# msracver/Relation-Networks-for-Object-Detection

Hardware: AMD Instinct MI355X
Metric: images/sec (1000x600, 300 ROIs) (higher is better)
Workload: dtype bf16; 1 GPU; BASELINE configs[1]: ResNet-101 Faster-RCNN + 2 relation modules (N=300, 16 heads, d=1024) + soft-NMS(0.6) + top-100, 600x1000 images, 300 proposals, random-init weights; launch=hipGraph replay, batches_in_flight=1, parallelism=replicas x1 (no data-path collective), ranks_seen_by_rccl=1

## Files before the change

include/relnet_hip.h:

```cpp
#ifndef RELNET_HIP_H
#define RELNET_HIP_H

#ifdef __cplusplus
extern "C" {
#endif

enum { RELNET_F32 = 0, RELNET_BF16 = 1 };

int relnet_version(void);
const char* relnet_last_error(void);
unsigned long long relnet_stream_capture_id(void* stream);

void _nms(int* keep_out, int* num_out, const float* boxes_host, int boxes_num, int boxes_dim,
          float nms_overlap_thresh, int device_id);

int relnet_proposal_decode(const float* cls_prob, const long* cls_strides4, const float* deltas,
                           const long* delta_strides4, const float* im_info, const double* base_anchors,
                           float* boxes , float* scores , int B, int A, int h, int w,
                           int feat_stride, int min_size, int softmax_pairs, void* stream);
int relnet_topk_sort(const float* scores, const float* boxes, float* out_boxes5, int* out_index,
                     int* out_count, int B, int n, int K, void* stream);
int relnet_nms_mask(const float* boxes5, const int* counts , unsigned long long* mask,
                    int B, int n, int n_stride, float thresh, void* stream);
int relnet_nms_scan(const unsigned long long* mask, const float* boxes5, const int* counts, float* rois,
// ... 73 lines not shown

int relnet_geometry_bias(const float* boxes, int box_stride, int box_off, const float* wp_t, const float* bp,
                         const float* divisors8, void* bias, int bias_half , float* pos_mat,
                         float* pos_emb, int B, int N, int M, int Mpad, int fc_dim, int nmod, void* stream);

int relnet_relation_attention(const void* q, long q_ld, long q_bs, const void* k, long k_ld, long k_bs,
                              const void* vwt, long vwt_ld, long vwt_bs, const void* bias, int bias_half,
                              long bias_bs, const float* bout, const void* resid, long resid_ld, long resid_bs, void* out,
                              long out_ld, long out_bs, void* out_act, long act_ld, long act_bs, float* logits,
                              int B, int H, int N, int M, int Mpad, float scale, int in_dtype, int out_dtype,
                              void* stream);

int relnet_relation_attention_kc(const void* q, long q_ld, long q_bs, const void* k, long k_ld, long k_bs,
                                 const void* vwt, long vwt_ld, long vwt_bs, const void* bias, int bias_half,
                                 long bias_bs, const float* bout, const void* resid, long resid_ld, long resid_bs, void* out,
                                 long out_ld, long out_bs, void* out_act, long act_ld, long act_bs, float* logits,
                                 int B, int H, int N, int M, int Mpad, float scale, int in_dtype, int out_dtype,
                                 const int* key_count, void* stream);
void relnet_relation_attention_debug_lds_f32(int on);

int relnet_relation_attention_fused(const void* q, long q_ld, long q_bs, const void* k, long k_ld, long k_bs,
                                    const void* vwt, long vwt_ld, long vwt_bs, const float* boxes, int box_stride,
                                    int box_off, const float* wp, const float* bp, const float* divisors8,
                                    const float* bout, const void* resid, long resid_ld, long resid_bs, void* out,
                                    long out_ld, long out_bs, void* out_act, long act_ld, long act_bs, int B, int H,
                                    int N, int M, int Mpad, float scale, void* stream);

int relnet_bottleneck_chain(const void* mid2, const void* x, const void* w3f, const void* w1f, const float* b3,
                            const float* b1, void* x_next, void* mid1_next, long P, int mid, void* stream);
int relnet_bottleneck_chain_proj(const void* mid2, const void* x_in, const void* w3f, const void* wpf, const void* w1f,
                                 const float* b3p, const float* b1, void* x_next, void* mid1_next, long P, int mid, void* stream);
int relnet_bottleneck_chain_s2(const void* mid2, const void* x, const void* w3f, const float* b3, void* x_next, int B, int H,
                               int W, int mid, void* stream);

int relnet_conv3x3_c64(const void* in, const void* w_frag, const float* bias, int relu, void* out, int B, int H, int W,
                       void* stream);
int relnet_conv3x3_c64_s2(const void* in, const void* w_frag, const float* bias, int relu, void* out, int B, int H, int W,
                          void* stream);


int relnet_pack_w_frag(const void* w, long ldw, void* out, int N, int K, void* stream);
int relnet_conv2d_nhwc_wf(const void* in, long in_pix, long in_img, const void* w, const void* w_frag, const float* bias,
                          const void* resid, int relu, void* out, long ldc, int B, int H, int W, int Cin, int Cout, int R,
                          int S, int stride, int dil, int pad, int out_dtype, void* stream);

int relnet_detect_head(const float* cls_score, long cs_ld, const float* bbox_pred, long bp_ld, const float* rois,
                       const float* im_info, float* cls_prob, double* boxes, int R, int C, int rois_per_image,
                       int delta_off, void* stream);
int relnet_detect_head_ex(const float* cls_score, long cs_ld, const float* bbox_pred, long bp_ld, const float* rois,
                          const float* im_info, float* cls_prob, double* boxes, int R, int C, int rois_per_image,
                          int delta_off, const int* n_valid, void* stream);
int relnet_class_nms(const float* cls_prob, const double* boxes, double* dets, int* counts, int B, int N, int C,
                     float score_thresh, double nms_param, int soft, int max_picks, void* stream);
int relnet_class_nms_ex(const float* cls_prob, const double* scores64, const double* boxes, double* dets, int* counts,
                        int* pick_index, int B, int N, int C, float score_thresh, double nms_param, int soft,
                        int max_picks, void* stream);
int relnet_class_nms_hist_bins(void);
int relnet_class_nms_topk(const float* cls_prob, const double* boxes, double* dets, int* counts, void* hist, int B, int N, int C,
                          float score_thresh, double nms_param, int soft, int max_picks, int top_k, void* stream);
int relnet_image_topk(const double* dets, const int* counts, double* thresh, int* total, float* out,
                      int* out_count, int B, int NC, int N, int max_per_image, int max_out, void* stream);

int relnet_lnms_prepare(const float* cls_score, long cs_ld, const float* bbox_pred, long bp_ld, const float* rois,
                        const float* im_info, float* prob , float* boxes , int B, int N,
                        int C, int delta_off, const float* means4, const float* stds4, void* stream);
int relnet_lnms_prepare_ex(const float* cls_score, long cs_ld, const float* bbox_pred, long bp_ld, const float* rois,
// ... 214 lines not shown
```

relation-networks-for-object-detection_amd/backbone.py:

```python
import math
import os

import torch
import torch.nn.functional as F

from . import ops

UNITS = (3, 4, 23, 3)
FILTERS = (256, 512, 1024, 2048)
EPS = 1e-5
PIXEL_MEANS = (103.06, 115.90, 123.15)


def unit_names(fpn=False):
    out = []
    in_ch = 64
    for si, (n, oc) in enumerate(zip(UNITS, FILTERS)):
        stage = si + 2
        for u in range(n):
            if n <= 3 or stage == 2 or stage == 5:
                name = 'abc'[u]
            else:
                name = 'a' if u == 0 else 'b%d' % u
            stride = 2 if (u == 0 and (stage in (3, 4) or (fpn and stage == 5))) else 1
# ... 51 lines not shown
        p['res5%s_branch2b_offset_weight' % u] = nrm(dcn_offset_std, 72, 512, 3, 3)
        p['res5%s_branch2b_offset_bias' % u] = torch.zeros(72)
    p['offset_weight'] = nrm(dcn_offset_std, 98, 256 * 49); p['offset_bias'] = torch.zeros(98)
    if fpn:
        for lvl, cin in ((32, 2048), (16, 1024), (8, 512), (4, 256)):
            p['fpn_ft%d_1x1_weight' % lvl] = nrm(0.01, 256, cin, 1, 1); p['fpn_ft%d_1x1_bias' % lvl] = torch.zeros(256)
            p['fpn_ft%d_3x3_weight' % lvl] = nrm(0.01, 256, 256, 3, 3); p['fpn_ft%d_3x3_bias' % lvl] = torch.zeros(256)
        p['fpn_ft64_3x3_weight'] = nrm(0.01, 256, 256, 3, 3); p['fpn_ft64_3x3_bias'] = torch.zeros(256)
        p['roi_pool_fc1_weight'] = nrm(0.01, 1024, 256 * 49); p['roi_pool_fc1_bias'] = torch.zeros(1024)
        p['roi_pool_fc2_weight'] = nrm(0.01, 1024, 1024); p['roi_pool_fc2_bias'] = torch.zeros(1024)
    return p


def fold_bn(w, gamma, beta, mean, var, eps=EPS):
    s = gamma.double() / torch.sqrt(var.double() + eps)
    return (w.double() * s.view(-1, 1, 1, 1)).float(), (beta.double() - mean.double() * s).float()


class Backbone(object):

    def __init__(self, params, dtype=torch.bfloat16, device='cuda', channels_last=True, impl=None, stem='hip', dcn=False,
                 fpn=False, chain=True, frozen_only=False, pixel_means=PIXEL_MEANS):
        self.dtype, self.device, self.dcn, self.fpn = dtype, device, dcn, fpn
        self.frozen_only = frozen_only
        self.pixel_means = tuple(float(v) for v in pixel_means)
        self.use_chain = chain
        env = os.environ.get('RELNET_STAGE_SPLIT')
        if env not in (None, '', '0'):
            self.stage_split = {int(a): int(b) for a, b in (kv.split(':') for kv in env.split(','))}
        if os.environ.get('RELNET_INPLACE_EXPAND') is not None:
            self.inplace_expand = os.environ['RELNET_INPLACE_EXPAND'] not in ('', '0')
        if os.environ.get('RELNET_QUARTER_UNITS') is not None:
            self.quarter_units = os.environ['RELNET_QUARTER_UNITS'] not in ('', '0')
        self.impl = impl or ('hip' if dtype == torch.bfloat16 else ('hip32' if dtype == torch.float32 and torch.device(device).type == 'cuda' else 'miopen'))
        if self.impl == 'hip' and torch.device(device).type == 'cuda':
            ops.asm_selfcheck()
        self.stem = stem
        assert self.impl in ('hip', 'hip32', 'miopen') and (self.impl != 'hip' or dtype == torch.bfloat16) and (self.impl != 'hip32' or dtype == torch.float32)
        self.mf = torch.channels_last if channels_last else torch.contiguous_format
        self.w = {}
        self.wp = {}
        self.wf = {}
        self.b32 = {}
        self.wp32 = {}
        for conv, bn, oc, ic, k in conv_bn_names():
            if frozen_only and not conv.startswith(('conv1', 'res2')):
                continue
            w, b = fold_bn(params[conv + '_weight'], params[bn + '_gamma'], params[bn + '_beta'],
                           params[bn + '_moving_mean'], params[bn + '_moving_var'])
            self._put(conv, w, b)
        if frozen_only:
            pass
        elif fpn:
            for lvl in (32, 16, 8, 4):
                for k in ('1x1', '3x3'):
                    name = 'fpn_ft%d_%s' % (lvl, k)
                    self._put(name, params[name + '_weight'], params[name + '_bias'])
        else:
            for name in ('rpn_conv_3x3', 'rpn_cls_score', 'rpn_bbox_pred', 'conv_new_1'):
                self._put(name, params[name + '_weight'], params[name + '_bias'])
            self._put('rpn_out', torch.cat([params['rpn_cls_score_weight'], params['rpn_bbox_pred_weight']], 0),
                      torch.cat([params['rpn_cls_score_bias'], params['rpn_bbox_pred_bias']], 0))
        self.units = [u for u in unit_names(fpn) if not frozen_only or u[0] == 2]
        self.wp_dcn = {}
        if dcn and not frozen_only:
            for u in 'abc':
# ... 54 lines not shown
    def _float_image(self, data, im_info, dtype):
        if data.dtype != torch.uint8:
            return data
        return ops.image_transform_u8(data, self.pixel_means, im_info, dtype=dtype)

    def forward_res2(self, data, im_info=None):
        if self.impl == 'hip32':
            assert self.frozen_only
            return self._forward_hip32(self._float_image(data, im_info, torch.float32))
        x = ops.stem_fused(data, self.w_stem, self.b32['conv1'], im_info, self.pixel_means)
        y_next = None
        self.last_chain_units = []
        for unit in self.units:
            if unit[0] != 2:
                break
            x, y_next = self._unit_hip(x, unit, y_next)
        return x

    def _forward_hip(self, data, rpn_hook=None, im_info=None):
        if self.stem == 'hip':
            x = ops.stem_fused(data, self.w_stem, self.b32['conv1'], im_info, self.pixel_means)
        elif self.stem == 'hip3':
            x = ops.stem_conv7(self._float_image(data, im_info, torch.float32), self.w_stem, self.b32['conv1'], relu=True)
            x = ops.stem_bias_relu_pool(x, self.zero_bias64)
        else:
            x = self._float_image(data, im_info, torch.float32).to(self.dtype).contiguous(memory_format=self.mf)
            x = F.conv2d(x, self.w['conv1'][0], None, stride=2, padding=3)
            x = ops.stem_bias_relu_pool(x.permute(0, 2, 3, 1), self.b32['conv1'])
        conv4 = None
        ends = {}
        y_next = None
        side, hooked = None, None
        self.last_chain_units, self.last_side_stream, self.last_stage_split = [], False, {}
        self.last_quarter_units = []
        compact = False
        ui = 0
        while ui < len(self.units):
            unit = self.units[ui]
            stage, proj = unit[0], unit[7]
            if stage == 5 and conv4 is None:
                conv4 = x
                if rpn_hook is not None and not self.fpn:
                    main = torch.cuda.current_stream()
                    side = self._side_stream()
                    self.last_side_stream = True
                    side.wait_stream(main)
                    with torch.cuda.stream(side):
                        hooked = self._rpn_head(conv4)
                        hooked = hooked + (rpn_hook(hooked[0], hooked[1]),)
            if proj and stage > 2:
                ends[stage - 1] = x
            nsplit = self._stage_split(stage, x, unit) if proj else 1
            if nsplit > 1:
                stage_units = [u for u in self.units if u[0] == stage]
                x = self._run_stage_split(x, stage_units, nsplit)
                ui += len(stage_units)
                continue
            quarter = self._quarter_ok(x, unit, self.units[ui + 1] if ui + 1 < len(self.units) else None)
            x, y_next = self._unit_hip(x, unit, y_next, inplace=self.inplace_expand, quarter=quarter, subsampled=compact)
            compact = quarter
            ui += 1
        conv5 = x
        nchw = lambda t: t.permute(0, 3, 1, 2)
        if self.fpn:
            tops = {32: self._hconv(conv5, 'fpn_ft32_1x1')}
            for lvl, src in ((16, ends[4]), (8, ends[3]), (4, ends[2])):
                tops[lvl] = ops.upsample2x_add_(self._hconv(src, 'fpn_ft%d_1x1' % lvl), tops[lvl * 2])
            out = {'fpn_ft%d' % lvl: nchw(self._hconv(tops[lvl], 'fpn_ft%d_3x3' % lvl, pad=1)) for lvl in (4, 8, 16, 32)}
            out.update(conv4=nchw(conv4), conv5=nchw(conv5))
            return out
        feat = self._hconv(conv5, 'conv_new_1', relu=True)
        out = dict(conv4=nchw(conv4), conv5=nchw(conv5), conv_new_1_relu=nchw(feat))
        if hooked is not None:
            torch.cuda.current_stream().wait_stream(side)
            out.update(rpn_cls_score=hooked[0], rpn_bbox_pred=hooked[1], rpn_hook=hooked[2])
        else:
            out['rpn_cls_score'], out['rpn_bbox_pred'] = self._rpn_head(conv4)
        return out

    stage_split = None
    inplace_expand = True

    quarter_units = True

    def _quarter_ok(self, x, unit, nxt):
        stage, nm, ic, mc, oc, stride, dil, proj = unit
        if not self.quarter_units or self.fpn or nxt is None or nxt[0] != stage + 1 or nxt[5] != 2 or not nxt[7]:
            return False
        ch = self.chain.get(nm)
        if ch is None or ch[1] is not None or mc not in ops.CHAIN_S2_MIDS or proj or dil != 1 or (self.dcn and stage == 5):
            return False
        if mc in ops.HALO3_CHANNELS and ('res%s_branch2b' % nm) not in self.halo3:
            return False
        if self.stage_split and (self._stage_split(stage, x, unit) > 1 or self._stage_split(nxt[0], x, nxt) > 1):
            return False
        B, H, W, C = x.shape
        return C == oc and x.numel() * 2 < (1 << 32) and ops.chain_worthwhile(B * ((H - 1) // 2 + 1) * ((W - 1) // 2 + 1), mc)

    def _stage_split(self, stage, x, unit):
        return int(self.stage_split.get(stage, 1)) if self.stage_split else 1

    def _run_stage_split(self, x, stage_units, nsplit):
        B = x.shape[0]
        stage = stage_units[0][0]
        st, nm, ic, mc, oc, stride, dil, proj = stage_units[0]
        Ho, Wo = (x.shape[1] - 1) // stride + 1, (x.shape[2] - 1) // stride + 1
        out = torch.empty((B, Ho, Wo, oc), device=x.device, dtype=x.dtype)
        bounds = [(B * i) // nsplit for i in range(nsplit + 1)]
        self.last_stage_split[stage] = [hi - lo for lo, hi in zip(bounds, bounds[1:])]
        for lo, hi in zip(bounds, bounds[1:]):
            xs, ys = x[lo:hi], None
            for unit in stage_units:
                xs, ys = self._unit_hip(xs, unit, ys, sc_out=out[lo:hi] if unit[7] else None, inplace=self.inplace_expand, force_chain=True)
            if xs.data_ptr() != out[lo:hi].data_ptr():
                out[lo:hi].copy_(xs)
        return out

    def _unit_hip(self, x, unit, y_pre=None, sc_out=None, inplace=False, force_chain=False, quarter=False, subsampled=False):
        stage, nm, ic, mc, oc, stride, dil, proj = unit
        if subsampled:
            assert stride == 2 and proj
            stride = 1
        if quarter:
            y = y_pre if y_pre is not None else self._hconv(x, 'res%s_branch2a' % nm, relu=True)
            if ('res%s_branch2b' % nm) in self.halo3:
                y = ops.conv3x3_halo_s2(y.contiguous(), *self.halo3['res%s_branch2b' % nm], relu=True)
            else:
                y = self._hconv(y, 'res%s_branch2b' % nm, stride=2, pad=1, relu=True)
            w3f, _, b3, _ = self.chain[nm]
            if nm not in self.last_chain_units:
                self.last_chain_units.append(nm)
            self.last_quarter_units.append(nm)
            return ops.bottleneck_chain_s2(y, x.contiguous(), w3f, b3), None
        fuse_proj = (nm in self.chain_proj and sc_out is None and x.is_contiguous()
                     and (force_chain or ops.chain_worthwhile(x.numel() // x.shape[-1], mc)))
        if fuse_proj:
            sc = None
        elif proj:
            w, b, k = self.wp['res%s_branch1' % nm]
            sc = ops.conv2d_nhwc(x, w, b, ksize=k, stride=stride, out=sc_out)
        else:
            sc = x
        y = y_pre if y_pre is not None else self._hconv(x, 'res%s_branch2a' % nm, stride=stride, relu=True)
        if self.dcn and stage == 5:
            y = self._deform_2b(y.permute(0, 3, 1, 2), 'res%s_branch2b' % nm,
                                self._hconv(y, 'res%s_branch2b_offset' % nm, pad=2, dil=2, out_dtype=torch.float32).permute(0, 3, 1, 2))
            y = y.permute(0, 2, 3, 1)
        elif ('res%s_branch2b' % nm) in self.halo3:
            y = ops.conv3x3_halo(y.contiguous(), *self.halo3['res%s_branch2b' % nm], relu=True)
        else:
            y = self._hconv(y, 'res%s_branch2b' % nm, pad=dil, dil=dil, relu=True)
        if fuse_proj:
            if nm not in self.last_chain_units:
                self.last_chain_units.append(nm)
            return ops.bottleneck_chain_proj(y, x, *self.chain_proj[nm])
        ch = self.chain.get(nm)
        if ch is not None and not force_chain and not ops.chain_worthwhile(y.numel() // y.shape[-1], y.shape[-1]):
            ch = None
        if ch is not None:
            if nm not in self.last_chain_units:
                self.last_chain_units.append(nm)
            return ops.bottleneck_chain(y, sc.contiguous(), *ch, inplace=inplace and sc.is_contiguous())
        return self._hconv(y, 'res%s_branch2c' % nm, relu=True, resid=sc), None

    def _rpn_head(self, conv4):
        r = self._hconv(conv4, 'rpn_conv_3x3', pad=1, relu=True)
        rpn = self._hconv(r, 'rpn_out', out_dtype=torch.float32)
        na2 = self.w['rpn_cls_score'][0].shape[0]
        return rpn[..., :na2].permute(0, 3, 1, 2), rpn[..., na2:].permute(0, 3, 1, 2)

    def _side_stream(self):
        if getattr(self, '_side', None) is None:
            self._side = torch.cuda.Stream(device=self.device)
        return self._side

    def _deform_2b(self, y, name, offset):
        w, b = self.wp_dcn[name]
        return ops.deformable_conv(y, offset, w, b, 3, 1, 2, 2, 4, relu=True)

    def _conv(self, x, name, stride=1, pad=0, dil=1, relu=False):
        w, b = self.w[name]
        y = F.conv2d(x, w, b, stride=stride, padding=pad, dilation=dil)
        return F.relu_(y) if relu else y

    def _c32(self, x, name, stride=1, pad=0, dil=1, relu=False, resid=None):
        w, b, k = self.wp32[name]
        return ops.conv2d_nhwc_f32(x, w, b, ksize=k, stride=stride, pad=pad, dil=dil, relu=relu, resid=resid)

    def _forward_hip32(self, data):
        B, Cin, H, W = data.shape
        x = torch.zeros((B, H, W, 16), device=data.device, dtype=torch.float32)
        x[..., :Cin] = data.permute(0, 2, 3, 1)
        x = self._c32(x, 'conv1', stride=2, pad=3, relu=True)
        x = ops.maxpool_nhwc_f32(x, 3, 2)
        conv4, ends = None, {}
# ... 70 lines not shown
```

relation-networks-for-object-detection_amd/csrc/bottleneck.hip:

```cpp
#include "common.h"

namespace relnet {

typedef const __attribute__((address_space(1))) void* gas_ptr;
typedef __attribute__((address_space(3))) void* las_ptr;

__device__ __forceinline__ void chain_glds16(const void* src, unsigned lds_byte_addr) {
  asm volatile("s_mov_b32 m0, %1\n\ts_nop 0\n\tglobal_load_lds_dwordx4 %0, off" ::"v"(src), "s"(lds_byte_addr) : "memory", "m0");
}

struct ChainArgs {
  const unsigned short* m2;
  const unsigned short* x;
  const uint4* w3f;
  const uint4* w1f;
  const float* b3;
  const float* b1;
  const unsigned short* xin;
  const uint4* wpf;
  unsigned short* xn;
  unsigned short* m1;
  int P;
  int H, W, Ho, Wo;
  int dbg;
};

template <int MID, bool STREAM, bool REDUCE = true, int KSPLIT = 1, bool PROJ = false, bool GATHER = false>
__global__ __launch_bounds__(512) void bottleneck_chain_kernel(ChainArgs a) {
  static_assert(!PROJ || (!STREAM && KSPLIT == 1), "the projection form exists for the resident-weight kernel");
  static_assert(!GATHER || (!REDUCE && !PROJ && KSPLIT == 1), "the stride-2 gather exists for the plain expand-only forms");
  static_assert(KSPLIT == 1 || (STREAM && !REDUCE), "k-split passes exist for the streamed expand-only form");
  constexpr int COUT = 4 * MID, KS = MID / 16, KSS = KS / KSPLIT, RT = MID / 32, NP = COUT / 64;
  static_assert(!REDUCE || MID <= 128, "MID = 256 with the second product is chain256_roles_kernel");
  constexpr int W3P = 2 * KSS * 1024, W1P = REDUCE ? 4 * RT * 1024 : 0;
  constexpr int WPP = PROJ ? W3P : 0;
  constexpr int PASSB = W3P + WPP + W1P;
  constexpr int STG = PROJ ? 4096 : 8192;
  constexpr int WBYTES = STREAM ? 2 * PASSB : NP * PASSB;
  extern __shared__ __attribute__((aligned(16))) unsigned char smem[];
  const int tid = threadIdx.x, lane = tid & 63;
  const int wave = __builtin_amdgcn_readfirstlane(tid >> 6);
  const int half = lane >> 5, l31 = lane & 31;
  unsigned char* stage = smem + WBYTES + wave * STG;
  float* sB3 = (float*)(smem + WBYTES + 8 * STG);
  float* sB1 = sB3 + COUT;
  for (int i = tid; i < COUT; i += 512) sB3[i] = a.b3[i];
  if constexpr (REDUCE) for (int i = tid; i < MID; i += 512) sB1[i] = a.b1[i];
  if constexpr (!STREAM) {
    for (int i = tid; i < NP * PASSB / 16; i += 512) {
      const int p = i / (PASSB / 16), r = i % (PASSB / 16);
      uint4 v;
      if (r < W3P / 16) v = a.w3f[(long)p * (W3P / 16) + r];
      else if (r < (W3P + WPP) / 16) v = a.wpf[(long)p * (W3P / 16) + (r - W3P / 16)];
      else { const int q = (r - (W3P + WPP) / 16) >> 6, rt = q >> 2, kk = q & 3; v = a.w1f[((long)rt * (COUT / 16) + p * 4 + kk) * 64 + (r & 63)]; }
      ((uint4*)smem)[i] = v;
    }
  }
  __syncthreads();
  const int ntile = (a.P + 31) / 32;
  const int drow = lane >> 3, dslot = lane & 7;
  unsigned xrow[GATHER ? 4 : 1];
  auto gather_rows = [&](int p0) {
    if constexpr (GATHER) {
      const unsigned hw = (unsigned)(a.Ho * a.Wo);
#pragma unroll
      for (int i = 0; i < 4; ++i) {
        const unsigned q = (unsigned)min(p0 + 8 * i + drow, a.P - 1);
        const unsigned b = q / hw, r = q - b * hw, yo = r / (unsigned)a.Wo, xo = r - yo * (unsigned)a.Wo;
        xrow[i] = ((b * (unsigned)a.H + 2u * yo) * (unsigned)a.W + 2u * xo) * (COUT * 2u);
      }
    }
  };
  auto issue_x = [&](int p0, int p) {
    if constexpr (PROJ) return;
    unsigned char* sb = stage + (p & 1) * 4096;
#pragma unroll
    for (int i = 0; i < 4; ++i) {
      const int row = 8 * i + drow;
      const unsigned off = GATHER ? xrow[i] + (p * 64 + ((dslot ^ ((row >> 1) & 7)) << 3)) * 2u
                                  : ((unsigned)min(p0 + row, a.P - 1) * COUT + p * 64 + ((dslot ^ ((row >> 1) & 7)) << 3)) * 2u;
      __builtin_amdgcn_global_load_lds((gas_ptr)((const unsigned char*)a.x + off), (las_ptr)(sb + i * 1024), 16, 0, 0);
    }
  };
  auto issue_w = [&](int st) {
    if constexpr (STREAM) {
      const int p = st / KSPLIT, kh = st % KSPLIT;
      unsigned char* wb = smem + (st & 1) * PASSB;
#pragma unroll
      for (int i = 0; i < (2 * KSS + (REDUCE ? 4 * RT : 0)) / 8; ++i) {
        const int q = wave + 8 * i;
        if (q < 2 * KSS) {
          const int ct = q / KSS, ks = q % KSS;
          __builtin_amdgcn_global_load_lds((gas_ptr)(a.w3f + ((long)((p * 2 + ct) * KS + kh * KSS + ks) * 64 + lane)), (las_ptr)(wb + q * 1024), 16, 0, 0);
        } else {
          const int q1 = q - 2 * KSS, rt = q1 >> 2, kk = q1 & 3;
          __builtin_amdgcn_global_load_lds((gas_ptr)(a.w1f + ((long)(rt * (COUT / 16) + p * 4 + kk) * 64 + lane)), (las_ptr)(wb + W3P + q1 * 1024), 16, 0, 0);
        }
      }
    }
  };
  auto flush = [&](int p0, int p) {
    const unsigned char* sb = stage + (PROJ ? 0 : (p & 1) * 4096) + lane * 16;
    const uint4 v0 = *(const uint4*)sb, v1 = *(const uint4*)(sb + 1024), v2 = *(const uint4*)(sb + 2048), v3 = *(const uint4*)(sb + 3072);
    asm volatile("s_waitcnt lgkmcnt(0)" ::: "memory");
    auto put = [&](int i, const uint4& v) {
      const int row = 8 * i + drow;
      if (p0 + row < a.P) *(uint4*)((unsigned char*)a.xn + ((unsigned)(p0 + row) * COUT + p * 64 + ((dslot ^ ((row >> 1) & 7)) << 3)) * 2u) = v;
    };
    put(0, v0); put(1, v1); put(2, v2); put(3, v3);
  };

  const int t_first = blockIdx.x * 8 + wave;
  const int t_step = gridDim.x * 8;
  const int n_iter = STREAM ? ((ntile + 7) / 8 - (int)blockIdx.x + (int)gridDim.x - 1) / (int)gridDim.x
                            : (ntile - t_first + t_step - 1) / t_step;
  if (n_iter <= 0) return;
  gather_rows(t_first * 32);
  issue_x(t_first * 32, 0);
  issue_w(0);
  for (int it = 0; it < n_iter; ++it) {
    const int p0 = (t_first + it * t_step) * 32;
    const int px = min(p0 + l31, a.P - 1);
    bf16x8 m2f[KS];
#pragma unroll
    for (int ks = 0; ks < KS; ++ks) m2f[ks] = *(const bf16x8*)(a.m2 + (long)px * MID + 16 * ks + 8 * half);
    bf16x8 xf[PROJ ? KS : 1];
    if constexpr (PROJ) {
#pragma unroll
      for (int ks = 0; ks < KS; ++ks) xf[ks] = *(const bf16x8*)(a.xin + (long)px * MID + 16 * ks + 8 * half);
    }
    f32x16 m1acc[RT];
#pragma unroll
    for (int rt = 0; rt < RT; ++rt)
#pragma unroll
      for (int r = 0; r < 16; ++r) m1acc[rt][r] = 0.f;
#pragma unroll 1
    for (int p = 0; p < NP; ++p) {
      f32x16 acc[2];
#pragma unroll
      for (int kh = 0; kh < KSPLIT; ++kh) {
        const int st = p * KSPLIT + kh;
        if constexpr (STREAM) asm volatile("s_waitcnt vmcnt(0)\n\ts_barrier" ::: "memory");
        else if constexpr (!PROJ) asm volatile("s_waitcnt vmcnt(0)" ::: "memory");
        if (kh == 0) {
          if (!PROJ && p > 0) flush(p0, p - 1);
          if (p + 1 < NP) issue_x(p0, p + 1);
          else if (it + 1 < n_iter) { gather_rows(p0 + t_step * 32); issue_x(p0 + t_step * 32, 0); }
        }
        if (st + 1 < NP * KSPLIT) issue_w(st + 1);
        else if (it + 1 < n_iter) issue_w(0);
        const uint4* w3 = (const uint4*)(smem + (STREAM ? (st & 1) : st) * PASSB);
#pragma unroll
        for (int ct = 0; ct < 2; ++ct) {
          if (kh == 0)
#pragma unroll
// ... 305 lines not shown
    else if (mid == 128) bottleneck_chain_kernel<128, true, false><<<grid, 512, lds, (hipStream_t)stream>>>(a);
    else if (mid == 256) bottleneck_chain_kernel<256, true, false><<<grid, 512, lds, (hipStream_t)stream>>>(a);
    else bottleneck_chain_kernel<512, true, false, 2><<<grid, 512, lds, (hipStream_t)stream>>>(a);
  }
  return check_launch("relnet_bottleneck_chain");
}

extern "C" int relnet_bottleneck_chain_s2(const void* mid2, const void* x, const void* w3f, const float* b3, void* x_next, int B,
                                          int H, int W, int mid, void* stream) {
  RELNET_REQUIRE(mid2 && x && w3f && b3 && x_next && x_next != x, "relnet_bottleneck_chain_s2: null operand (or x_next == x: this form is never in place)");
  RELNET_REQUIRE(mid == 64 || mid == 128, "relnet_bottleneck_chain_s2: mid = %d unsupported (64, 128)", mid);
  RELNET_REQUIRE(B > 0 && H > 0 && W > 0 && (long)B * H * W * 8 * mid < (1L << 32),
                 "relnet_bottleneck_chain_s2: bad geometry B=%d H=%d W=%d (the full 4 mid-channel map must stay below 4 GiB)", B, H, W);
  ChainArgs a;
  a.m2 = (const unsigned short*)mid2; a.x = (const unsigned short*)x; a.w3f = (const uint4*)w3f; a.w1f = nullptr;
  a.b3 = b3; a.b1 = nullptr; a.xn = (unsigned short*)x_next; a.m1 = nullptr;
  a.xin = nullptr; a.wpf = nullptr; a.dbg = 0;
  a.H = H; a.W = W; a.Ho = (H - 1) / 2 + 1; a.Wo = (W - 1) / 2 + 1;
  const long P = (long)B * a.Ho * a.Wo;
  a.P = (int)P;
  static relnet::PerDeviceOnce attr_once;
  if (attr_once.first()) {
    hipFuncSetAttribute((const void*)bottleneck_chain_kernel<64, false, false, 1, false, true>, hipFuncAttributeMaxDynamicSharedMemorySize, 160 * 1024);
    hipFuncSetAttribute((const void*)bottleneck_chain_kernel<128, true, false, 1, false, true>, hipFuncAttributeMaxDynamicSharedMemorySize, 160 * 1024);
  }
  const long ntile = (P + 31) / 32;
  const unsigned grid = (unsigned)(ntile < 8 * 256 ? (ntile + 7) / 8 : 256);
  const size_t lds = 65536 + 65536 + (size_t)5 * mid * 4;
  if (mid == 64) bottleneck_chain_kernel<64, false, false, 1, false, true><<<grid, 512, lds, (hipStream_t)stream>>>(a);
  else bottleneck_chain_kernel<128, true, false, 1, false, true><<<grid, 512, lds, (hipStream_t)stream>>>(a);
  return check_launch("relnet_bottleneck_chain_s2");
}

extern "C" int relnet_bottleneck_chain_proj(const void* mid2, const void* x_in, const void* w3f, const void* wpf, const void* w1f,
                                            const float* b3p, const float* b1, void* x_next, void* mid1_next, long P, int mid,
                                            void* stream) {
  RELNET_REQUIRE(mid2 && x_in && w3f && wpf && b3p && x_next, "relnet_bottleneck_chain_proj: null operand");
  RELNET_REQUIRE((w1f && b1 && mid1_next) || (!w1f && !b1 && !mid1_next), "relnet_bottleneck_chain_proj: w1f, b1 and mid1_next are given together (or all NULL)");
  RELNET_REQUIRE(mid == 64, "relnet_bottleneck_chain_proj: mid = %d unsupported (64)", mid);
  RELNET_REQUIRE(P > 0 && P * 8 * mid < (1L << 32), "relnet_bottleneck_chain_proj: bad pixel count %ld (x_next is addressed with 32-bit byte offsets: the 4 mid-channel map must stay below 4 GiB)", P);
  ChainArgs a;
  a.m2 = (const unsigned short*)mid2; a.x = nullptr; a.w3f = (const uint4*)w3f; a.w1f = (const uint4*)w1f;
  a.b3 = b3p; a.b1 = b1; a.xn = (unsigned short*)x_next; a.m1 = (unsigned short*)mid1_next; a.P = (int)P;
  a.xin = (const unsigned short*)x_in; a.wpf = (const uint4*)wpf; a.dbg = 0;
  a.H = a.W = a.Ho = a.Wo = 0;
  static relnet::PerDeviceOnce attr_once;
  if (attr_once.first()) {
    hipFuncSetAttribute((const void*)bottleneck_chain_kernel<64, false, true, 1, true>, hipFuncAttributeMaxDynamicSharedMemorySize, 160 * 1024);
    hipFuncSetAttribute((const void*)bottleneck_chain_kernel<64, false, false, 1, true>, hipFuncAttributeMaxDynamicSharedMemorySize, 160 * 1024);
  }
  const long ntile = (P + 31) / 32;
  const unsigned grid = (unsigned)(ntile < 8 * 256 ? (ntile + 7) / 8 : 256);
  const size_t lds = (size_t)4 * (8192 + 8192 + (mid1_next ? 8192 : 0)) + 8 * 4096 + (size_t)5 * mid * 4;
  if (mid1_next) bottleneck_chain_kernel<64, false, true, 1, true><<<grid, 512, lds, (hipStream_t)stream>>>(a);
  else bottleneck_chain_kernel<64, false, false, 1, true><<<grid, 512, lds, (hipStream_t)stream>>>(a);
  return check_launch("relnet_bottleneck_chain_proj");
}

namespace relnet {

__device__ __attribute__((aligned(16))) const unsigned int g_zero_chunk[4] = {0u, 0u, 0u, 0u};

struct Halo3Args {
  const unsigned short* in;
  const uint4* wf;
  const float* bias;
// ... 178 lines not shown
```

relation-networks-for-object-detection_amd/lib.py:

```python
import ctypes as C
import os
import sys

HERE = os.path.dirname(os.path.abspath(__file__))
LIB_PATH = os.environ.get('RELNET_LIB') or os.path.join(HERE, 'librelnet_hip.so')

F32, BF16 = 0, 1


class RelnetError(RuntimeError):
    pass


_lib = None

_vp, _i, _l, _f, _d = C.c_void_p, C.c_int, C.c_long, C.c_float, C.c_double

_SIGNATURES = {
    'relnet_version': (C.c_int, []),
    'relnet_last_error': (C.c_char_p, []),
    'relnet_gemm_nt': (C.c_int, [_vp, _l, _l, _vp, _l, _l, _vp, _l, _l, _vp, _i, _vp, _i,
                                 _i, _i, _i, _i, _i, _i, _vp]),
    'relnet_geometry_bias': (C.c_int, [_vp, _i, _i, _vp, _vp, _vp, _vp, _i, _vp, _vp, _i, _i, _i, _i,
                                       _i, _i, _vp]),
    'relnet_relation_attention': (C.c_int, [_vp, _l, _l, _vp, _l, _l, _vp, _l, _l, _vp, _i, _l, _vp,
                                            _vp, _l, _l, _vp, _l, _l, _vp, _l, _l, _vp,
                                            _i, _i, _i, _i, _i, _f, _i, _i, _vp]),
    'relnet_relation_attention_kc': (C.c_int, [_vp, _l, _l, _vp, _l, _l, _vp, _l, _l, _vp, _i, _l, _vp,
                                               _vp, _l, _l, _vp, _l, _l, _vp, _l, _l, _vp,
                                               _i, _i, _i, _i, _i, _f, _i, _i, _vp, _vp]),
    'relnet_relation_attention_fused': (C.c_int, [_vp, _l, _l, _vp, _l, _l, _vp, _l, _l, _vp, _i, _i, _vp, _vp, _vp,
                                                  _vp, _vp, _l, _l, _vp, _l, _l, _vp, _l, _l,
                                                  _i, _i, _i, _i, _i, _f, _vp]),
    'relnet_bottleneck_chain': (C.c_int, [_vp, _vp, _vp, _vp, _vp, _vp, _vp, _vp, _l, _i, _vp]),
    'relnet_bottleneck_chain_proj': (C.c_int, [_vp, _vp, _vp, _vp, _vp, _vp, _vp, _vp, _vp, _l, _i, _vp]),
    'relnet_conv3x3_c64': (C.c_int, [_vp, _vp, _vp, _i, _vp, _i, _i, _i, _vp]),
    'relnet_conv3x3_c64_s2': (C.c_int, [_vp, _vp, _vp, _i, _vp, _i, _i, _i, _vp]),
    'relnet_bottleneck_chain_s2': (C.c_int, [_vp, _vp, _vp, _vp, _vp, _i, _i, _i, _i, _vp]),
    'relnet_proposal_decode': (C.c_int, [_vp, _vp, _vp, _vp, _vp, _vp, _vp, _vp, _i, _i, _i, _i, _i, _i, _i, _vp]),
    'relnet_topk_sort': (C.c_int, [_vp, _vp, _vp, _vp, _vp, _i, _i, _i, _vp]),
    'relnet_nms_mask': (C.c_int, [_vp, _vp, _vp, _i, _i, _i, _f, _vp]),
    'relnet_nms_scan': (C.c_int, [_vp, _vp, _vp, _vp, _vp, _vp, _vp, _i, _i, _i, _i, _i, _i, _vp]),
    '_nms': (None, [_vp, _vp, _vp, _i, _i, _f, _i]),
    'relnet_roi_pool_fwd': (C.c_int, [_vp, _vp, _vp, _vp, _vp, _vp, _i, _i, _i, _i, _i, _i, _f, _i, _i, _vp]),
    'relnet_roi_align_fwd': (C.c_int, [_vp, _vp, _vp, _vp, _vp, _i, _i, _i, _i, _i, _i, _f, _i, _i, _i, _i, _vp]),
    'relnet_roi_align_bwd': (C.c_int, [_vp, _vp, _vp, _vp, _vp, _i, _i, _i, _i, _i, _i, _f, _i, _i, _i, _i, _vp]),
    'relnet_roi_align_levels_fwd': (C.c_int, [_vp, _vp, _vp, _vp, _vp, _i, _vp, _vp, _vp, _vp] + [_i] * 9 + [_vp]),
    'relnet_roi_align_levels_bwd': (C.c_int, [_vp, _vp, _vp, _vp, _vp, _vp, _vp, _vp, _vp] + [_i] * 10 + [_vp]),
    'relnet_roi_pool_bwd': (C.c_int, [_vp, _vp, _vp, _vp, _vp, _l, _l, _i, _i, _i, _i, _i, _i, _i, _vp]),
    'relnet_roi_pool_bwd_ex': (C.c_int, [_vp, _vp, _vp, _vp, _vp, _l, _l, _l, _i, _i, _i, _i, _i, _i, _i, _vp]),
    'relnet_roi_pool_fpn_bwd_ex': (C.c_int, [_vp, _vp, _vp, _vp, _vp, _vp, _vp, _vp, _vp, _i, _i, _i, _i, _i, _i, _i, _vp]),
    'relnet_detect_head': (C.c_int, [_vp, _l, _vp, _l, _vp, _vp, _vp, _vp, _i, _i, _i, _i, _vp]),
    'relnet_detect_head_ex': (C.c_int, [_vp, _l, _vp, _l, _vp, _vp, _vp, _vp, _i, _i, _i, _i, _vp, _vp]),
    'relnet_class_nms': (C.c_int, [_vp, _vp, _vp, _vp, _i, _i, _i, _f, C.c_double, _i, _i, _vp]),
    'relnet_class_nms_ex': (C.c_int, [_vp, _vp, _vp, _vp, _vp, _vp, _i, _i, _i, _f, C.c_double, _i, _i, _vp]),
    'relnet_class_nms_topk': (C.c_int, [_vp, _vp, _vp, _vp, _vp, _i, _i, _i, _f, C.c_double, _i, _i, _i, _vp]),
    'relnet_class_nms_hist_bins': (C.c_int, []),
    'relnet_bbox_overlaps': (C.c_int, [_vp, _vp, _vp, _i, _i, _vp]),
    'relnet_image_topk': (C.c_int, [_vp, _vp, _vp, _vp, _vp, _vp, _i, _i, _i, _i, _i, _vp]),
    'relnet_conv2d_nhwc': (C.c_int, [_vp, _l, _l, _vp, _vp, _vp, _i, _vp, _l, _i, _i, _i, _i, _i, _i, _i, _i, _i, _i, _i, _vp]),
    'relnet_conv2d_nhwc_f32': (C.c_int, [_vp, _l, _l, _vp, _vp, _vp, _i, _vp, _l, _i, _i, _i, _i, _i, _i, _i, _i, _i, _i, _vp]),
    'relnet_maxpool_nhwc_f32': (C.c_int, [_vp, _vp, _i, _i, _i, _i, _i, _i, _vp]),
    'relnet_pack_w_frag': (C.c_int, [_vp, _l, _vp, _i, _i, _vp]),
    'relnet_conv2d_nhwc_wf': (C.c_int, [_vp, _l, _l, _vp, _vp, _vp, _vp, _i, _vp, _l, _i, _i, _i, _i, _i, _i, _i, _i, _i, _i, _i, _vp]),
    'relnet_deformable_im2col': (C.c_int, [_vp, _vp, _vp, _vp, _vp, _l] + [_i] * 15 + [_vp]),
    'relnet_deformable_psroi_pool_fwd': (C.c_int, [_vp, _vp, _vp, _vp, _vp, _vp, _vp] + [_i] * 9 + [_f, _f, _i, _i, _i, _vp]),
    'relnet_roi_pool_fpn_fwd': (C.c_int, [_vp, _vp, _vp, _vp, _vp, _i, _vp, _vp, _vp, _vp, _vp, _i, _i, _i, _i, _i, _i, _vp]),
    'relnet_fpn_roi_dispatch': (C.c_int, [_vp, _i, _i, _vp, _vp, _vp, _vp, _i, _i, _i, _vp]),
    'relnet_fpn_roi_dispatch_ex': (C.c_int, [_vp, _i, _i, _vp, _vp, _vp, _vp, _i, _i, _i, _vp, _i, _i, _vp, _vp]),
    'relnet_upsample2x_add': (C.c_int, [_vp, _vp, _i, _i, _i, _i, _i, _vp]),
    'relnet_softmax_output': (C.c_int, [_vp, _vp, _vp, _vp, _vp, _l, _i, _l, _i, _f, _f, _vp]),
# ... 149 lines not shown
```

relation-networks-for-object-detection_amd/ops.py:

```python
import math
import os

import torch

from . import lib as _lib

F32, BF16 = _lib.F32, _lib.BF16


def _dt(t):
    if t.dtype == torch.float32:
        return F32
    if t.dtype == torch.bfloat16:
        return BF16
    raise TypeError("unsupported dtype %s (float32 or bfloat16)" % t.dtype)


def _chk(*ts):
    for t in ts:
        if t is not None:
            if not t.is_cuda:
                raise _lib.RelnetError("relnet ops need GPU tensors (HIP kernels only; no CPU fallback)")


# ... 565 lines not shown
    row = rt * 32 + (lane & 31)
    col = ks * 16 + 8 * (t >> 2) + 4 * (lane >> 5) + (t & 3)
    return w_packed[row, col].contiguous()


def bottleneck_chain(mid2, x, w3_frag, w1_frag, b3, b1, inplace=False):
    _chk(mid2, x, w3_frag, w1_frag, b3, b1)
    mid = mid2.shape[-1]
    assert mid2.is_contiguous() and x.is_contiguous() and x.shape[-1] == 4 * mid and x.shape[:-1] == mid2.shape[:-1]
    assert mid2.dtype == torch.bfloat16 and x.dtype == torch.bfloat16 and b3.dtype == torch.float32
    assert (w1_frag is None) == (b1 is None) and (b1 is None or b1.dtype == torch.float32)
    assert mid in (CHAIN_MIDS if w1_frag is not None else CHAIN_EXPAND_MIDS)
    xn = x if inplace else torch.empty_like(x)
    m1 = torch.empty_like(mid2) if w1_frag is not None else None
    _lib.call('relnet_bottleneck_chain', mid2.data_ptr(), x.data_ptr(), w3_frag.data_ptr(), _ptr(w1_frag), b3.data_ptr(),
              _ptr(b1), xn.data_ptr(), _ptr(m1), mid2.numel() // mid, mid, _stream())
    return xn, m1


CHAIN_S2_MIDS = (64, 128)


def bottleneck_chain_s2(mid2, x, w3_frag, b3):
    _chk(mid2, x, w3_frag, b3)
    mid = mid2.shape[-1]
    B, H, W, C = x.shape
    assert mid in CHAIN_S2_MIDS and C == 4 * mid and mid2.shape == (B, (H - 1) // 2 + 1, (W - 1) // 2 + 1, mid)
    assert mid2.is_contiguous() and x.is_contiguous() and x.numel() * 2 < (1 << 32)
    assert mid2.dtype == torch.bfloat16 and x.dtype == torch.bfloat16 and b3.dtype == torch.float32
    xn = torch.empty(mid2.shape[:-1] + (C,), device=x.device, dtype=x.dtype)
    _lib.call('relnet_bottleneck_chain_s2', mid2.data_ptr(), x.data_ptr(), w3_frag.data_ptr(), b3.data_ptr(), xn.data_ptr(), B, H, W, mid,
              _stream())
    return xn


def bottleneck_chain_proj(mid2, x_in, w3_frag, wp_frag, w1_frag, b3p, b1):
    _chk(mid2, x_in, w3_frag, wp_frag, w1_frag, b3p, b1)
    mid = mid2.shape[-1]
    assert mid == 64 and x_in.shape == mid2.shape and mid2.is_contiguous() and x_in.is_contiguous()
    assert mid2.dtype == torch.bfloat16 and x_in.dtype == torch.bfloat16 and b3p.dtype == torch.float32
    assert (w1_frag is None) == (b1 is None)
    xn = torch.empty(mid2.shape[:-1] + (4 * mid,), device=mid2.device, dtype=torch.bfloat16)
    m1 = torch.empty_like(mid2) if w1_frag is not None else None
    _lib.call('relnet_bottleneck_chain_proj', mid2.data_ptr(), x_in.data_ptr(), w3_frag.data_ptr(), wp_frag.data_ptr(), _ptr(w1_frag),
              b3p.data_ptr(), _ptr(b1), xn.data_ptr(), _ptr(m1), mid2.numel() // mid, mid, _stream())
    return xn, m1


def conv2d_nhwc(x, w_packed, bias, ksize=1, stride=1, pad=0, dil=1, relu=False, resid=None, out=None,
                out_dtype=None, w_frag=None):
    _chk(x, w_packed, bias, resid, out)
    if x.dtype == torch.float32:
        return conv2d_nhwc_f32(x, w_packed, bias, ksize, stride, pad, dil, relu, resid, out)
    assert x.dtype == torch.bfloat16 and w_packed.dtype == torch.bfloat16 and x.stride(3) == 1
    B, H, W, Cin = x.shape
    assert x.stride(1) == W * x.stride(2), "rows of an image must be dense in W"
    Cout = w_packed.shape[0]
    assert w_packed.shape[1] == ksize * ksize * Cin and w_packed.is_contiguous()
    Hout = (H + 2 * pad - dil * (ksize - 1) - 1) // stride + 1
    Wout = (W + 2 * pad - dil * (ksize - 1) - 1) // stride + 1
    odt = out_dtype or (out.dtype if out is not None else x.dtype)
    if out is None:
        out = torch.empty((B, Hout, Wout, Cout), device=x.device, dtype=odt)
    assert out.shape == (B, Hout, Wout, Cout) and out.stride(3) == 1
    assert out.stride(1) == Wout * out.stride(2) and out.stride(0) == Hout * out.stride(1)
    if resid is not None:
# ... 745 lines not shown
```

Before: 2983 images/s.

## Store only even-pixel outputs from the chain kernel preceding a stride-2 quarter unit

Adds an EVEN variant of the fused bottleneck chain kernel. When the following unit is a stride-2 quarter unit, it writes the expanded output x_next only at even (y,x) pixels into a compact subsampled map, while still producing the full mid1 map for the next unit. The next quarter unit then reads this compact map as its shortcut through the plain chain kernel instead of gathering it with stride 2. The intent is to cut three quarters of the full-resolution write of the 4*mid-channel activation and the strided gather that followed it. In exchange the kernel does extra per-row index arithmetic, and the Python scheduling becomes more coupled because each unit now depends on the two units after it.

```diff
diff --git a/include/relnet_hip.h b/include/relnet_hip.h
--- a/include/relnet_hip.h
+++ b/include/relnet_hip.h
@@ -129,6 +129,8 @@
                                  const float* b3p, const float* b1, void* x_next, void* mid1_next, long P, int mid, void* stream);
 int relnet_bottleneck_chain_s2(const void* mid2, const void* x, const void* w3f, const float* b3, void* x_next, int B, int H,
                                int W, int mid, void* stream);
+int relnet_bottleneck_chain_even(const void* mid2, const void* x, const void* w3f, const void* w1f, const float* b3, const float* b1,
+                                 void* x_next_even, void* mid1_next, int B, int H, int W, int mid, void* stream);
 
 int relnet_conv3x3_c64(const void* in, const void* w_frag, const float* bias, int relu, void* out, int B, int H, int W,
                        void* stream);
diff --git a/relation-networks-for-object-detection_amd/backbone.py b/relation-networks-for-object-detection_amd/backbone.py
--- a/relation-networks-for-object-detection_amd/backbone.py
+++ b/relation-networks-for-object-detection_amd/backbone.py
@@ -107,6 +107,8 @@
             self.inplace_expand = os.environ['RELNET_INPLACE_EXPAND'] not in ('', '0')
         if os.environ.get('RELNET_QUARTER_UNITS') is not None:
             self.quarter_units = os.environ['RELNET_QUARTER_UNITS'] not in ('', '0')
+        if os.environ.get('RELNET_EVEN_STORE') is not None:
+            self.even_store = os.environ['RELNET_EVEN_STORE'] not in ('', '0')
         self.impl = impl or ('hip' if dtype == torch.bfloat16 else ('hip32' if dtype == torch.float32 and torch.device(device).type == 'cuda' else 'miopen'))
         if self.impl == 'hip' and torch.device(device).type == 'cuda':
             ops.asm_selfcheck()
@@ -227,8 +229,9 @@
         y_next = None
         side, hooked = None, None
         self.last_chain_units, self.last_side_stream, self.last_stage_split = [], False, {}
-        self.last_quarter_units = []
+        self.last_quarter_units, self.last_even_store_units = [], []
         compact = False
+        even_prev = False
         ui = 0
         while ui < len(self.units):
             unit = self.units[ui]
@@ -251,9 +254,12 @@
                 x = self._run_stage_split(x, stage_units, nsplit)
                 ui += len(stage_units)
                 continue
-            quarter = self._quarter_ok(x, unit, self.units[ui + 1] if ui + 1 < len(self.units) else None)
-            x, y_next = self._unit_hip(x, unit, y_next, inplace=self.inplace_expand, quarter=quarter, subsampled=compact)
-            compact = quarter
+            after = lambda k: self.units[ui + k] if ui + k < len(self.units) else None
+            quarter = even_prev or self._quarter_ok(x, unit, after(1))
+            even = not quarter and self._even_store_ok(x, unit, after(1), after(2))
+            x, y_next = self._unit_hip(x, unit, y_next, inplace=self.inplace_expand, quarter=quarter, subsampled=compact,
+                                       even_store=even, compact_shortcut=even_prev)
+            compact, even_prev = quarter, even
             ui += 1
         conv5 = x
         nchw = lambda t: t.permute(0, 3, 1, 2)
@@ -292,6 +298,17 @@
         B, H, W, C = x.shape
         return C == oc and x.numel() * 2 < (1 << 32) and ops.chain_worthwhile(B * ((H - 1) // 2 + 1) * ((W - 1) // 2 + 1), mc)
 
+    even_store = True
+
+    def _even_store_ok(self, x, unit, nxt, nxt2):
+        stage, nm, ic, mc, oc, stride, dil, proj = unit
+        if not self.even_store or proj or nxt is None or nxt[0] != stage or not self._quarter_ok(x, nxt, nxt2):
+            return False
+        ch = self.chain.get(nm)
+        if ch is None or ch[1] is None or mc not in ops.CHAIN_S2_MIDS or dil != 1 or not x.is_contiguous():
+            return False
+        return ops.chain_worthwhile(x.numel() // x.shape[-1], mc)
+
     def _stage_split(self, stage, x, unit):
         return int(self.stage_split.get(stage, 1)) if self.stage_split else 1
 
@@ -311,12 +328,14 @@
                 out[lo:hi].copy_(xs)
         return out
 
-    def _unit_hip(self, x, unit, y_pre=None, sc_out=None, inplace=False, force_chain=False, quarter=False, subsampled=False):
+    def _unit_hip(self, x, unit, y_pre=None, sc_out=None, inplace=False, force_chain=False, quarter=False, subsampled=False,
+                  even_store=False, compact_shortcut=False):
         stage, nm, ic, mc, oc, stride, dil, proj = unit
         if subsampled:
             assert stride == 2 and proj
             stride = 1
         if quarter:
+            assert y_pre is not None or not compact_shortcut
             y = y_pre if y_pre is not None else self._hconv(x, 'res%s_branch2a' % nm, relu=True)
             if ('res%s_branch2b' % nm) in self.halo3:
                 y = ops.conv3x3_halo_s2(y.contiguous(), *self.halo3['res%s_branch2b' % nm], relu=True)
@@ -326,6 +345,8 @@
             if nm not in self.last_chain_units:
                 self.last_chain_units.append(nm)
             self.last_quarter_units.append(nm)
+            if compact_shortcut:
+                return ops.bottleneck_chain(y, x, w3f, None, b3, None)[0], None
             return ops.bottleneck_chain_s2(y, x.contiguous(), w3f, b3), None
         fuse_proj = (nm in self.chain_proj and sc_out is None and x.is_contiguous()
                      and (force_chain or ops.chain_worthwhile(x.numel() // x.shape[-1], mc)))
@@ -355,7 +376,11 @@
         if ch is not None:
             if nm not in self.last_chain_units:
                 self.last_chain_units.append(nm)
+            if even_store:
+                self.last_even_store_units.append(nm)
+                return ops.bottleneck_chain_even(y, sc, *ch)
             return ops.bottleneck_chain(y, sc.contiguous(), *ch, inplace=inplace and sc.is_contiguous())
+        assert not even_store
         return self._hconv(y, 'res%s_branch2c' % nm, relu=True, resid=sc), None
 
     def _rpn_head(self, conv4):
diff --git a/relation-networks-for-object-detection_amd/csrc/bottleneck.hip b/relation-networks-for-object-detection_amd/csrc/bottleneck.hip
--- a/relation-networks-for-object-detection_amd/csrc/bottleneck.hip
+++ b/relation-networks-for-object-detection_amd/csrc/bottleneck.hip
@@ -25,10 +25,11 @@
   int dbg;
 };
 
-template <int MID, bool STREAM, bool REDUCE = true, int KSPLIT = 1, bool PROJ = false, bool GATHER = false>
+template <int MID, bool STREAM, bool REDUCE = true, int KSPLIT = 1, bool PROJ = false, bool GATHER = false, bool EVEN = false>
 __global__ __launch_bounds__(512) void bottleneck_chain_kernel(ChainArgs a) {
   static_assert(!PROJ || (!STREAM && KSPLIT == 1), "the projection form exists for the resident-weight kernel");
   static_assert(!GATHER || (!REDUCE && !PROJ && KSPLIT == 1), "the stride-2 gather exists for the plain expand-only forms");
+  static_assert(!EVEN || (REDUCE && !PROJ && !GATHER && KSPLIT == 1), "the even-pixel x_next exists for the plain two-product forms");
   static_assert(KSPLIT == 1 || (STREAM && !REDUCE), "k-split passes exist for the streamed expand-only form");
   constexpr int COUT = 4 * MID, KS = MID / 16, KSS = KS / KSPLIT, RT = MID / 32, NP = COUT / 64;
   static_assert(!REDUCE || MID <= 128, "MID = 256 with the second product is chain256_roles_kernel");
@@ -71,6 +72,20 @@
       }
     }
   };
+  constexpr unsigned kDropped = 0xffffffffu;
+  unsigned erow[EVEN ? 4 : 1];
+  auto even_rows = [&](int p0) {
+    if constexpr (EVEN) {
+      const unsigned hw = (unsigned)(a.H * a.W);
+#pragma unroll
+      for (int i = 0; i < 4; ++i) {
+        const unsigned q = (unsigned)(p0 + 8 * i + drow);
+        const unsigned b = q / hw, r = q - b * hw, y = r / (unsigned)a.W, xx = r - y * (unsigned)a.W;
+        const bool keep = q < (unsigned)a.P && !((y | xx) & 1u);
+        erow[i] = keep ? ((b * (unsigned)a.Ho + (y >> 1)) * (unsigned)a.Wo + (xx >> 1)) * (COUT * 2u) : kDropped;
+      }
+    }
+  };
   auto issue_x = [&](int p0, int p) {
     if constexpr (PROJ) return;
     unsigned char* sb = stage + (p & 1) * 4096;
@@ -105,7 +120,11 @@
     asm volatile("s_waitcnt lgkmcnt(0)" ::: "memory");
     auto put = [&](int i, const uint4& v) {
       const int row = 8 * i + drow;
-      if (p0 + row < a.P) *(uint4*)((unsigned char*)a.xn + ((unsigned)(p0 + row) * COUT + p * 64 + ((dslot ^ ((row >> 1) & 7)) << 3)) * 2u) = v;
+      if constexpr (EVEN) {
+        if (p0 + row < a.P && erow[i] != kDropped) *(uint4*)((unsigned char*)a.xn + (erow[i] + (p * 64 + ((dslot ^ ((row >> 1) & 7)) << 3)) * 2u)) = v;
+      } else {
+        if (p0 + row < a.P) *(uint4*)((unsigned char*)a.xn + ((unsigned)(p0 + row) * COUT + p * 64 + ((dslot ^ ((row >> 1) & 7)) << 3)) * 2u) = v;
+      }
     };
     put(0, v0); put(1, v1); put(2, v2); put(3, v3);
   };
@@ -121,6 +140,7 @@
   for (int it = 0; it < n_iter; ++it) {
     const int p0 = (t_first + it * t_step) * 32;
     const int px = min(p0 + l31, a.P - 1);
+    even_rows(p0);
     bf16x8 m2f[KS];
 #pragma unroll
     for (int ks = 0; ks < KS; ++ks) m2f[ks] = *(const bf16x8*)(a.m2 + (long)px * MID + 16 * ks + 8 * half);
@@ -492,6 +512,34 @@
   return check_launch("relnet_bottleneck_chain_s2");
 }
 
+extern "C" int relnet_bottleneck_chain_even(const void* mid2, const void* x, const void* w3f, const void* w1f, const float* b3,
+                                            const float* b1, void* x_next_even, void* mid1_next, int B, int H, int W, int mid,
+                                            void* stream) {
+  RELNET_REQUIRE(mid2 && x && w3f && b3 && x_next_even && x_next_even != x, "relnet_bottleneck_chain_even: null operand (or x_next_even == x: this form is never in place)");
+  RELNET_REQUIRE(w1f && b1 && mid1_next, "relnet_bottleneck_chain_even: w1f, b1 and mid1_next are required (the expand-only form at the even pixels is relnet_bottleneck_chain_s2)");
+  RELNET_REQUIRE(mid == 64 || mid == 128, "relnet_bottleneck_chain_even: mid = %d unsupported (64, 128)", mid);
+  RELNET_REQUIRE(B > 0 && H > 0 && W > 0 && (long)B * H * W * 8 * mid < (1L << 32),
+                 "relnet_bottleneck_chain_even: bad geometry B=%d H=%d W=%d (the full 4 mid-channel map must stay below 4 GiB)", B, H, W);
+  ChainArgs a;
+  a.m2 = (const unsigned short*)mid2; a.x = (const unsigned short*)x; a.w3f = (const uint4*)w3f; a.w1f = (const uint4*)w1f;
+  a.b3 = b3; a.b1 = b1; a.xn = (unsigned short*)x_next_even; a.m1 = (unsigned short*)mid1_next;
+  a.xin = nullptr; a.wpf = nullptr; a.dbg = 0;
+  a.H = H; a.W = W; a.Ho = (H - 1) / 2 + 1; a.Wo = (W - 1) / 2 + 1;
+  const long P = (long)B * H * W;
+  a.P = (int)P;
+  static relnet::PerDeviceOnce attr_once;
+  if (attr_once.first()) {
+    hipFuncSetAttribute((const void*)bottleneck_chain_kernel<64, false, true, 1, false, false, true>, hipFuncAttributeMaxDynamicSharedMemorySize, 160 * 1024);
+    hipFuncSetAttribute((const void*)bottleneck_chain_kernel<128, true, true, 1, false, false, true>, hipFuncAttributeMaxDynamicSharedMemorySize, 160 * 1024);
+  }
+  const long ntile = (P + 31) / 32;
+  const unsigned grid = (unsigned)(ntile < 8 * 256 ? (ntile + 7) / 8 : 256);
+  const size_t lds = 65536 + 65536 + (size_t)5 * mid * 4;
+  if (mid == 64) bottleneck_chain_kernel<64, false, true, 1, false, false, true><<<grid, 512, lds, (hipStream_t)stream>>>(a);
+  else bottleneck_chain_kernel<128, true, true, 1, false, false, true><<<grid, 512, lds, (hipStream_t)stream>>>(a);
+  return check_launch("relnet_bottleneck_chain_even");
+}
+
 extern "C" int relnet_bottleneck_chain_proj(const void* mid2, const void* x_in, const void* w3f, const void* wpf, const void* w1f,
                                             const float* b3p, const float* b1, void* x_next, void* mid1_next, long P, int mid,
                                             void* stream) {
diff --git a/relation-networks-for-object-detection_amd/lib.py b/relation-networks-for-object-detection_amd/lib.py
--- a/relation-networks-for-object-detection_amd/lib.py
+++ b/relation-networks-for-object-detection_amd/lib.py
@@ -37,6 +37,7 @@
     'relnet_conv3x3_c64': (C.c_int, [_vp, _vp, _vp, _i, _vp, _i, _i, _i, _vp]),
     'relnet_conv3x3_c64_s2': (C.c_int, [_vp, _vp, _vp, _i, _vp, _i, _i, _i, _vp]),
     'relnet_bottleneck_chain_s2': (C.c_int, [_vp, _vp, _vp, _vp, _vp, _i, _i, _i, _i, _vp]),
+    'relnet_bottleneck_chain_even': (C.c_int, [_vp, _vp, _vp, _vp, _vp, _vp, _vp, _vp, _i, _i, _i, _i, _vp]),
     'relnet_proposal_decode': (C.c_int, [_vp, _vp, _vp, _vp, _vp, _vp, _vp, _vp, _i, _i, _i, _i, _i, _i, _i, _vp]),
     'relnet_topk_sort': (C.c_int, [_vp, _vp, _vp, _vp, _vp, _i, _i, _i, _vp]),
     'relnet_nms_mask': (C.c_int, [_vp, _vp, _vp, _i, _i, _i, _f, _vp]),
diff --git a/relation-networks-for-object-detection_amd/ops.py b/relation-networks-for-object-detection_amd/ops.py
--- a/relation-networks-for-object-detection_amd/ops.py
+++ b/relation-networks-for-object-detection_amd/ops.py
@@ -621,6 +621,23 @@
     _lib.call('relnet_bottleneck_chain_s2', mid2.data_ptr(), x.data_ptr(), w3_frag.data_ptr(), b3.data_ptr(), xn.data_ptr(), B, H, W, mid,
               _stream())
     return xn
+
+
+def bottleneck_chain_even(mid2, x, w3_frag, w1_frag, b3, b1, out=None):
+    _chk(mid2, x, w3_frag, w1_frag, b3, b1, out)
+    mid = mid2.shape[-1]
+    B, H, W, C = x.shape
+    assert mid in CHAIN_S2_MIDS and C == 4 * mid and mid2.shape == (B, H, W, mid)
+    assert mid2.is_contiguous() and x.is_contiguous() and x.numel() * 2 < (1 << 32)
+    assert mid2.dtype == torch.bfloat16 and x.dtype == torch.bfloat16 and b3.dtype == torch.float32 and b1.dtype == torch.float32
+    shape = (B, (H - 1) // 2 + 1, (W - 1) // 2 + 1, C)
+    if out is None:
+        out = torch.empty(shape, device=x.device, dtype=x.dtype)
+    assert tuple(out.shape) == shape and out.is_contiguous() and out.dtype == x.dtype and out.data_ptr() != x.data_ptr()
+    m1 = torch.empty_like(mid2)
+    _lib.call('relnet_bottleneck_chain_even', mid2.data_ptr(), x.data_ptr(), w3_frag.data_ptr(), w1_frag.data_ptr(), b3.data_ptr(),
+              b1.data_ptr(), out.data_ptr(), m1.data_ptr(), B, H, W, mid, _stream())
+    return out, m1
 
 
 def bottleneck_chain_proj(mid2, x_in, w3_frag, wp_frag, w1_frag, b3p, b1):
```

Result: no change. 2997 images/s, median of 6 (+0.5%).
